# UofgCoastline/EUSIPCO-2026-Robust-Unet

Hardware: NVIDIA B200
Metric: train_images_per_sec (higher is better)
Workload: dtype bf16

## Files before the change

### eusipco-2026-robust-unet_b200/csrc/wgrad_gemm.cu

```cuda
#include "rbu_common.cuh"
#include "rbu_ptx.cuh"
#include "tma_host.cuh"
#include <stdlib.h>

namespace {

constexpr int TILE_PX = 128;
constexpr int BOX_BYTES = TILE_PX * 128;
constexpr int NUM_THREADS = 192;
constexpr int A_STAGES = 2;
constexpr int SMEM_LIMIT = 232448;

struct WParams {
  int N, H, W;
  int TW, TH, TN;
  int tiles_w, tiles_h, tiles_n, tiles_total;
  int Mtot, Ntot, taps, dil, gather;
  int tap_first, tap_end;
  int BM, BN, T;
  int m_blocks, n_blocks, t_groups, ksplit, items;
  int b_stages, tmem_cols;
  float* partial;
};

__device__ __forceinline__ void decode_item(const WParams& p, int item, int& mb, int& nb, int& tg, int& ks) {
  mb = item % p.m_blocks; item /= p.m_blocks;
  nb = item % p.n_blocks; item /= p.n_blocks;
  tg = item % p.t_groups;
  ks = item / p.t_groups;
}
__device__ __forceinline__ void tile_origin(const WParams& p, int tile, int& w0, int& h0, int& n0) {
  w0 = (tile % p.tiles_w) * p.TW;
  tile /= p.tiles_w;
  h0 = (tile % p.tiles_h) * p.TH;
  n0 = (tile / p.tiles_h) * p.TN;
}

__global__ void __launch_bounds__(NUM_THREADS, 1)
wgrad_gemm_kernel(const __grid_constant__ CUtensorMap tmA, const __grid_constant__ CUtensorMap tmB,
                  const __grid_constant__ WParams p) {
  extern __shared__ uint8_t smem_raw[];
  uint8_t* smem = reinterpret_cast<uint8_t*>((reinterpret_cast<uintptr_t>(smem_raw) + 1023) & ~uintptr_t(1023));
  const int a_boxes = p.BM / 64 > 0 ? (p.BM + 63) / 64 : 1;
  const int b_boxes = (p.BN + 63) / 64;
  const int a_bytes = a_boxes * BOX_BYTES;
  const int b_bytes = b_boxes * BOX_BYTES;
  uint8_t* smA = smem;
  uint8_t* smB = smem + A_STAGES * a_bytes;
  uint64_t* bars = reinterpret_cast<uint64_t*>(smB + p.b_stages * b_bytes);
  uint64_t* fullA = bars;
  uint64_t* emptyA = bars + 2;
  uint64_t* fullB = bars + 4;
  uint64_t* emptyB = bars + 12;
  uint64_t* tfull = bars + 20;
  uint64_t* tempty = bars + 21;
  uint32_t* tmem_slot = reinterpret_cast<uint32_t*>(bars + 22);

  const int warp = threadIdx.x >> 5, lane = threadIdx.x & 31;
  if (warp == 0 && lane == 0) {
    ptx::prefetch_tmap(&tmA);
    ptx::prefetch_tmap(&tmB);
  }
  if (warp == 1 && lane == 0) {
    for (int s = 0; s < A_STAGES; ++s) { ptx::mbar_init(&fullA[s], 1); ptx::mbar_init(&emptyA[s], 1); }
    for (int s = 0; s < p.b_stages; ++s) { ptx::mbar_init(&fullB[s], 1); ptx::mbar_init(&emptyB[s], 1); }
    ptx::mbar_init(tfull, 1);
    ptx::mbar_init(tempty, 4);
    ptx::fence_barrier_init();
  }
  if (warp == 2) {
    ptx::tmem_alloc(tmem_slot, (uint32_t)p.tmem_cols);
    ptx::tmem_relinquish();
  }
  ptx::tc_fence_before();
  __syncthreads();
  ptx::tc_fence_after();
  const uint32_t tmem_base = *tmem_slot;

  if (warp == 0) {
    if (lane == 0) {
      int sa = 0, sb = 0;
      uint32_t pha = 0, phb = 0;
      for (int item = blockIdx.x; item < p.items; item += gridDim.x) {
        int mb, nb, tg, ks;
        decode_item(p, item, mb, nb, tg, ks);
        const int t_begin = p.tap_first + tg * p.T;
        const int t_end = min(t_begin + p.T, p.tap_end);
        const int tile0 = (int)((long)ks * p.tiles_total / p.ksplit);
        const int tile1 = (int)((long)(ks + 1) * p.tiles_total / p.ksplit);
        for (int tile = tile0; tile < tile1; ++tile) {
          int w0, h0, n0;
          tile_origin(p, tile, w0, h0, n0);
          {
            const int s = sa;
            const uint32_t ph = pha;
            if (++sa == A_STAGES) { sa = 0; pha ^= 1; }
            ptx::mbar_wait(&emptyA[s], ph ^ 1);
            ptx::mbar_arrive_expect_tx(&fullA[s], (uint32_t)a_bytes);
            for (int bx = 0; bx < a_boxes; ++bx)
              ptx::tma_load_4d(smA + s * a_bytes + bx * BOX_BYTES, &tmA, &fullA[s], mb * p.BM + bx * 64, w0, h0, n0);
          }
          for (int t = t_begin; t < t_end; ++t) {
            const int s = sb;
            const uint32_t ph = phb;
            if (++sb == p.b_stages) { sb = 0; phb ^= 1; }
            ptx::mbar_wait(&emptyB[s], ph ^ 1);
            ptx::mbar_arrive_expect_tx(&fullB[s], (uint32_t)b_bytes);
            for (int bx = 0; bx < b_boxes; ++bx) {
              uint8_t* dst = smB + s * b_bytes + bx * BOX_BYTES;
              const int c0 = nb * p.BN + bx * 64;
              if (p.gather) {
                ptx::tma_load_5d(dst, &tmB, &fullB[s], c0, t & 1, w0, t >> 1, h0);
              } else {
                int dh = 0, dw = 0;
                if (p.taps == 9) { dh = (t / 3 - 1) * p.dil; dw = (t % 3 - 1) * p.dil; }
                ptx::tma_load_4d(dst, &tmB, &fullB[s], c0, w0 + dw, h0 + dh, n0);
              }
            }
          }
        }
      }
    }
  } else if (warp == 1) {
    const uint32_t idesc = ptx::make_idesc_bf16(p.BM, p.BN, 1, 1);
    const uint32_t fullA_s = ptx::smem_u32(fullA), emptyA_s = ptx::smem_u32(emptyA);
    const uint32_t fullB_s = ptx::smem_u32(fullB), emptyB_s = ptx::smem_u32(emptyB);
    const uint32_t hi = ptx::desc_hi(1024);
    const uint32_t a_lo0 = ptx::desc_lo(ptx::smem_u32(smA), BOX_BYTES), b_lo0 = ptx::desc_lo(ptx::smem_u32(smB), BOX_BYTES);
    const uint32_t a_step = (uint32_t)a_bytes >> 4, b_step = (uint32_t)b_bytes >> 4;
    int sa = 0, sb = 0, it = 0;
    uint32_t pha = 0, phb = 0;
    for (int item = blockIdx.x; item < p.items; item += gridDim.x, ++it) {
      int mb, nb, tg, ks;
      decode_item(p, item, mb, nb, tg, ks);
      const int ntap = min(p.tap_first + tg * p.T + p.T, p.tap_end) - (p.tap_first + tg * p.T);
      const int tile0 = (int)((long)ks * p.tiles_total / p.ksplit);
      const int tile1 = (int)((long)(ks + 1) * p.tiles_total / p.ksplit);
      ptx::mbar_wait(tempty, (it & 1) ^ 1);
      ptx::tc_fence_after();
      uint32_t accumulate = 0;
      for (int tile = tile0; tile < tile1; ++tile) {
        ptx::mbar_wait_s(fullA_s + sa * 8, pha);
        ptx::tc_fence_after();
        const uint32_t a_lo = a_lo0 + sa * a_step;
        for (int t = 0; t < ntap; ++t) {
          ptx::mbar_wait_s(fullB_s + sb * 8, phb);
          ptx::tc_fence_after();
          if (ptx::elect_one()) {
            const uint32_t b_lo = b_lo0 + sb * b_step;
            const uint32_t d_tmem = tmem_base + (uint32_t)(t * p.BN);
#pragma unroll
            for (int k = 0; k < TILE_PX / 16; ++k)
              ptx::umma_bf16(d_tmem, ptx::pack_desc(a_lo + k * (2048 >> 4), hi), ptx::pack_desc(b_lo + k * (2048 >> 4), hi),
                             idesc, (k > 0) ? 1u : accumulate);
            ptx::umma_commit_s(emptyB_s + sb * 8);
          }
          __syncwarp();
          if (++sb == p.b_stages) { sb = 0; phb ^= 1; }
        }
        accumulate = 1;
        if (ptx::elect_one()) ptx::umma_commit_s(emptyA_s + sa * 8);
        __syncwarp();
        if (++sa == A_STAGES) { sa = 0; pha ^= 1; }
      }
      if (ptx::elect_one()) ptx::umma_commit(tfull);
      __syncwarp();
    }
  } else {
    const int lg = warp & 3;
    int it = 0;
    for (int item = blockIdx.x; item < p.items; item += gridDim.x, ++it) {
      int mb, nb, tg, ks;
      decode_item(p, item, mb, nb, tg, ks);
      const int t_begin = p.tap_first + tg * p.T;
      const int t_end = min(t_begin + p.T, p.tap_end);
      int m_local;
      bool row_ok;
      if (p.BM == 128) { m_local = lg * 32 + lane; row_ok = true; }
      else { m_local = lg * 16 + lane; row_ok = lane < 16; }
      const int m = mb * p.BM + m_local;
      row_ok = row_ok && (m < p.Mtot);
      ptx::mbar_wait(tfull, it & 1);
      ptx::tc_fence_after();
      const uint32_t t_addr = tmem_base + ((uint32_t)(lg * 32) << 16);
      for (int t = t_begin; t < t_end; ++t) {
        for (int c0 = 0; c0 < p.BN; c0 += 32) {
          uint32_t r[32];
          ptx::tmem_ld_32x32(t_addr + (uint32_t)((t - t_begin) * p.BN + c0), r);
          ptx::tmem_ld_wait();
          const int n0 = nb * p.BN + c0;
          if (row_ok && n0 < p.Ntot) {
            float* dst = p.partial + (((long)ks * p.Mtot + m) * p.taps + t) * p.Ntot + n0;
            if (n0 + 32 <= p.Ntot && (p.Ntot & 3) == 0) {
#pragma unroll
              for (int g = 0; g < 8; ++g)
                *reinterpret_cast<float4*>(dst + g * 4) = make_float4(__uint_as_float(r[g * 4]), __uint_as_float(r[g * 4 + 1]),
                                                                      __uint_as_float(r[g * 4 + 2]), __uint_as_float(r[g * 4 + 3]));
            } else {
              for (int e = 0; e < 32; ++e)
                if (n0 + e < p.Ntot) dst[e] = __uint_as_float(r[e]);
            }
          }
        }
      }
      ptx::tc_fence_before();
      __syncwarp();
      if (lane == 0) ptx::mbar_arrive(tempty);
    }
  }
  ptx::tc_fence_before();
  __syncthreads();
  if (warp == 2) ptx::tmem_dealloc(tmem_base, (uint32_t)p.tmem_cols);
}

template <int NCH>
__global__ void __launch_bounds__(256)
wgrad_reduce_kernel(const float* __restrict__ partial, int ksplit, int Mtot, int taps, int Ntot,
                    float* __restrict__ out, int accumulate, int tap_first, int tap_end) {
  constexpr int KL = 256 / NCH;
  constexpr int MAXT = 9;
  __shared__ float lane_sum[KL][MAXT][NCH + 1];
  __shared__ float res[NCH * MAXT];
  const int nchunks = (Ntot + NCH - 1) / NCH;
  const int m = blockIdx.x / nchunks, n0 = (blockIdx.x - m * nchunks) * NCH;
  const int nn = threadIdx.x % NCH, kl = threadIdx.x / NCH;
  const int n = n0 + nn;
  const long total = (long)Mtot * taps * Ntot;
  float acc[MAXT][2];
#pragma unroll
  for (int t = 0; t < MAXT; ++t) acc[t][0] = acc[t][1] = 0.f;
  if (n < Ntot) {
    const float* src = partial + (long)m * taps * Ntot + n;
    int k = kl;
    for (; k + KL < ksplit; k += 2 * KL) {
#pragma unroll
      for (int t = 0; t < MAXT; ++t)
        if (t >= tap_first && t < tap_end) {
          acc[t][0] += __ldg(src + (long)k * total + (long)t * Ntot);
          acc[t][1] += __ldg(src + (long)(k + KL) * total + (long)t * Ntot);
        }
    }
    if (k < ksplit) {
#pragma unroll
      for (int t = 0; t < MAXT; ++t)
        if (t >= tap_first && t < tap_end) acc[t][0] += __ldg(src + (long)k * total + (long)t * Ntot);
    }
  }
#pragma unroll
  for (int t = 0; t < MAXT; ++t)
    if (t < taps) lane_sum[kl][t][nn] = acc[t][0] + acc[t][1];
  __syncthreads();
  for (int i = threadIdx.x; i < NCH * taps; i += 256) {
    const int t = i / NCH, c = i - t * NCH;
    float sum = lane_sum[0][t][c];
    for (int j = 1; j < KL; ++j) sum += lane_sum[j][t][c];
    res[c * taps + t] = sum;
  }
  __syncthreads();
  const int nw = min(NCH, Ntot - n0);
  float* o = out + ((long)m * Ntot + n0) * taps;
  for (int i = threadIdx.x; i < nw * taps; i += 256) {
    const int t = i % taps;
    if (t >= tap_first && t < tap_end) o[i] = accumulate ? o[i] + res[i] : res[i];
  }
}

bool use_halo(const rbu_wgrad_args* a) {
  static int no_halo = -1;
  if (no_halo < 0) no_halo = getenv("RBU_NO_HALO") ? 1 : 0;
  return !no_halo && rbu_wgrad_halo_supported(a);
}

int pow2ceil_w(int v) {
  int r = 1;
  while (r < v) r <<= 1;
  return r;
}

struct Plan {
  WParams p;
  size_t ws_bytes;
};

int make_plan(const rbu_wgrad_args* a, Plan* pl, int tap_first = 0, int tap_end = -1) {
  WParams& p = pl->p;
  memset(&p, 0, sizeof(p));
  p.tap_first = tap_first;
  p.tap_end = tap_end < 0 ? a->taps : tap_end;
  p.N = a->N; p.H = a->H; p.W = a->W;
  p.gather = a->gather;
  p.taps = a->taps;
  p.dil = a->taps == 9 ? a->dil : 0;
  p.Mtot = a->Ca;
  p.Ntot = a->Cb;
  p.TW = pow2ceil_w(a->W) < 16 ? pow2ceil_w(a->W) : 16;
  if (a->gather) {
    p.TH = TILE_PX / p.TW;
    p.TN = 1;
    p.tiles_w = rbu_cdiv(a->W, p.TW);
    p.tiles_h = rbu_cdiv((long)a->N * a->H, p.TH);
    p.tiles_n = 1;
  } else {
    const int th_max = TILE_PX / p.TW;
    p.TH = pow2ceil_w(a->H) < th_max ? pow2ceil_w(a->H) : th_max;
    p.TN = TILE_PX / (p.TW * p.TH);
    p.tiles_w = rbu_cdiv(a->W, p.TW);
    p.tiles_h = rbu_cdiv(a->H, p.TH);
    p.tiles_n = rbu_cdiv(a->N, p.TN);
  }
  p.tiles_total = p.tiles_w * p.tiles_h * p.tiles_n;
  p.BM = a->Ca > 64 ? 128 : 64;
  p.BN = a->Cb > 64 ? 128 : 64;
  p.T = a->taps == 9 ? 3 : a->taps;
  p.m_blocks = rbu_cdiv(a->Ca, p.BM);
  p.n_blocks = rbu_cdiv(a->Cb, p.BN);
  p.t_groups = rbu_cdiv(p.tap_end - p.tap_first, p.T);
  const int base_items = p.m_blocks * p.n_blocks * p.t_groups;
  int ks = rbu_cdiv(2L * rbu_num_sms(), base_items);
  if (ks > p.tiles_total) ks = p.tiles_total;
  if (ks < 1) ks = 1;
  p.ksplit = ks;
  p.items = base_items * ks;
  const int a_bytes = ((p.BM + 63) / 64) * BOX_BYTES, b_bytes = ((p.BN + 63) / 64) * BOX_BYTES;
  p.b_stages = (SMEM_LIMIT - 2048 - A_STAGES * a_bytes) / b_bytes;
  if (p.b_stages > 8) p.b_stages = 8;
  p.tmem_cols = 32;
  while (p.tmem_cols < p.T * p.BN) p.tmem_cols <<= 1;
  pl->ws_bytes = (size_t)ks * a->Ca * a->taps * a->Cb * sizeof(float);
  return 0;
}

int check_args(const rbu_wgrad_args* a) {
  RBU_CHECK_ARG(a != nullptr, "rbu_wgrad_gemm: null args");
  RBU_CHECK_ARG(a->N > 0 && a->H > 0 && a->W > 0, "rbu_wgrad_gemm: bad pixel grid");
  RBU_CHECK_ARG(a->Ca > 0 && a->Ca % 8 == 0 && a->Cb > 0 && a->Cb % 8 == 0, "rbu_wgrad_gemm: channel counts must be multiples of 8");
  RBU_CHECK_ARG(a->a_ld % 8 == 0 && a->b_ld % 8 == 0, "rbu_wgrad_gemm: ld must be a multiple of 8");
  if (a->gather) RBU_CHECK_ARG(a->taps == 4, "rbu_wgrad_gemm: gather needs taps == 4");
  else RBU_CHECK_ARG(a->taps == 1 || (a->taps == 9 && a->dil >= 1), "rbu_wgrad_gemm: taps must be 1 or 9 (dil >= 1)");
  return RBU_OK;
}

}

void rbu_wgrad_reduce_launch(const float* partial, int ksplit, int Mtot, int taps, int Ntot, float* out, int accumulate,
                             cudaStream_t stream, int tap_first, int tap_end) {
  if (tap_end < 0) tap_end = taps;
  if (Ntot >= 64 && ksplit <= 16)
    wgrad_reduce_kernel<64><<<Mtot * ((Ntot + 63) / 64), 256, 0, stream>>>(partial, ksplit, Mtot, taps, Ntot, out, accumulate, tap_first, tap_end);
  else if (Ntot >= 32 && ksplit <= 64)
    wgrad_reduce_kernel<32><<<Mtot * ((Ntot + 31) / 32), 256, 0, stream>>>(partial, ksplit, Mtot, taps, Ntot, out, accumulate, tap_first, tap_end);
  else
    wgrad_reduce_kernel<16><<<Mtot * ((Ntot + 15) / 16), 256, 0, stream>>>(partial, ksplit, Mtot, taps, Ntot, out, accumulate, tap_first, tap_end);
}

extern "C" size_t rbu_wgrad_workspace_bytes(const rbu_wgrad_args* a) {
  if (check_args(a) != RBU_OK) return 0;
  if (use_halo(a)) return rbu_wgrad_halo_workspace_bytes(a);
  Plan pl;
  make_plan(a, &pl);
  return pl.ws_bytes;
}

size_t rbu_wgrad_generic_workspace_bytes(const rbu_wgrad_args* a, int tap_first, int tap_end) {
  Plan pl;
  make_plan(a, &pl, tap_first, tap_end);
  return pl.ws_bytes;
}

int rbu_wgrad_generic_launch(const rbu_wgrad_args* a, int tap_first, int tap_end, void* workspace, size_t workspace_bytes,
                             cudaStream_t stream) {
  int rc;
  Plan pl;
  make_plan(a, &pl, tap_first, tap_end);
  WParams& p = pl.p;
  RBU_CHECK_ARG(workspace && workspace_bytes >= pl.ws_bytes && ((uintptr_t)workspace & 15) == 0,
                "rbu_wgrad_gemm: workspace too small (%zu < %zu)", workspace_bytes, pl.ws_bytes);
  p.partial = reinterpret_cast<float*>(workspace);

  CUtensorMap tmA, tmB;
  {
    uint64_t dims[4], str[3];
    uint32_t box[4];
    dims[0] = (uint64_t)a->Ca;
    str[0] = (uint64_t)a->a_ld * 2;
    dims[1] = (uint64_t)a->W;
    box[0] = 64; box[1] = (uint32_t)p.TW; box[2] = (uint32_t)p.TH; box[3] = (uint32_t)p.TN;
    if (a->gather) {
      dims[2] = (uint64_t)a->N * a->H; dims[3] = 1;
      str[1] = (uint64_t)a->a_ld * 2 * a->W;
      str[2] = str[1] * dims[2];
    } else {
      dims[2] = (uint64_t)a->H; dims[3] = (uint64_t)a->N;
      str[1] = (uint64_t)a->a_ld * 2 * a->W;
      str[2] = str[1] * a->H;
    }
    rc = rbu_encode_tmap_bf16(&tmA, a->a, 4, dims, str, box);
    if (rc) return rc;
  }
  if (a->gather) {
    const uint64_t dims[5] = {(uint64_t)a->Cb, 2, (uint64_t)a->W, 2, (uint64_t)a->N * a->H};
    const uint64_t str[4] = {(uint64_t)a->b_ld * 2, (uint64_t)a->b_ld * 4, (uint64_t)a->b_ld * 2 * (2 * a->W),
                             (uint64_t)a->b_ld * 4 * (2 * a->W)};
    const uint32_t box[5] = {64, 1, (uint32_t)p.TW, 1, (uint32_t)p.TH};
    rc = rbu_encode_tmap_bf16(&tmB, a->b, 5, dims, str, box);
  } else {
    const uint64_t dims[4] = {(uint64_t)a->Cb, (uint64_t)a->W, (uint64_t)a->H, (uint64_t)a->N};
    const uint64_t str[3] = {(uint64_t)a->b_ld * 2, (uint64_t)a->b_ld * 2 * a->W, (uint64_t)a->b_ld * 2 * a->W * a->H};
    const uint32_t box[4] = {64, (uint32_t)p.TW, (uint32_t)p.TH, (uint32_t)p.TN};
    rc = rbu_encode_tmap_bf16(&tmB, a->b, 4, dims, str, box);
  }
  if (rc) return rc;

  const int a_bytes = ((p.BM + 63) / 64) * BOX_BYTES, b_bytes = ((p.BN + 63) / 64) * BOX_BYTES;
  const int smem_bytes = A_STAGES * a_bytes + p.b_stages * b_bytes + 1024 + 256;
  static std::atomic<unsigned long long> attr_set{0};
  if (rbu_first_use_on_device(&attr_set))
    RBU_CHECK_CUDA(cudaFuncSetAttribute(wgrad_gemm_kernel, cudaFuncAttributeMaxDynamicSharedMemorySize, SMEM_LIMIT));
  const int grid = p.items < rbu_num_sms() ? p.items : rbu_num_sms();
  wgrad_gemm_kernel<<<grid, NUM_THREADS, smem_bytes, stream>>>(tmA, tmB, p);
  RBU_CHECK_LAUNCH();
  rbu_wgrad_reduce_launch(p.partial, p.ksplit, p.Mtot, p.taps, p.Ntot, a->out, a->accumulate, stream, p.tap_first, p.tap_end);
  RBU_CHECK_LAUNCH();
  return RBU_OK;
}

extern "C" int rbu_wgrad_gemm(const rbu_wgrad_args* a, void* workspace, size_t workspace_bytes, void* stream_) {
  cudaStream_t stream = reinterpret_cast<cudaStream_t>(stream_);
  int rc = check_args(a);
  if (rc) return rc;
  RBU_CHECK_ARG(a->a && a->b && a->out && ((uintptr_t)a->a & 15) == 0 && ((uintptr_t)a->b & 15) == 0,
                "rbu_wgrad_gemm: null or misaligned pointer");
  if (use_halo(a)) {
    RBU_CHECK_ARG(workspace && workspace_bytes >= rbu_wgrad_halo_workspace_bytes(a) && ((uintptr_t)workspace & 15) == 0,
                  "rbu_wgrad_gemm: workspace too small");
    return rbu_wgrad_halo_launch(a, workspace, stream);
  }
  return rbu_wgrad_generic_launch(a, 0, -1, workspace, workspace_bytes, stream);
}
```

Before: 1809.

## Double-buffer wgrad TMEM accumulators, widen BN, add direct store, vectorize reduce

The weight-gradient GEMM now keeps two TMEM accumulator slots when they fit, so the epilogue can drain one item while the MMA warp fills the next. It also allows BN=256 with a retuned tap grouping. When split-K is 1 it writes straight to the output and skips both the partial workspace and the reduce kernel. The reduce kernel switches to float4 loads, 64 threads and dynamic shared memory. Risks: the BN=256 tile together with the ksplit heuristic (still computed from the old item count) may leave SMs idle, and the direct path writes to the output with strided scalar stores when taps>1.

```diff
diff --git a/eusipco-2026-robust-unet_b200/csrc/wgrad_gemm.cu b/eusipco-2026-robust-unet_b200/csrc/wgrad_gemm.cu
--- a/eusipco-2026-robust-unet_b200/csrc/wgrad_gemm.cu
+++ b/eusipco-2026-robust-unet_b200/csrc/wgrad_gemm.cu
@@ -20,7 +20,10 @@
   int BM, BN, T;
   int m_blocks, n_blocks, t_groups, ksplit, items;
   int b_stages, tmem_cols;
+  int slots;
+  int direct, accumulate;
   float* partial;
+  float* out;
 };
 
 __device__ __forceinline__ void decode_item(const WParams& p, int item, int& mb, int& nb, int& tg, int& ks) {
@@ -53,8 +56,8 @@
   uint64_t* fullB = bars + 4;
   uint64_t* emptyB = bars + 12;
   uint64_t* tfull = bars + 20;
-  uint64_t* tempty = bars + 21;
-  uint32_t* tmem_slot = reinterpret_cast<uint32_t*>(bars + 22);
+  uint64_t* tempty = bars + 22;
+  uint32_t* tmem_slot = reinterpret_cast<uint32_t*>(bars + 24);
 
   const int warp = threadIdx.x >> 5, lane = threadIdx.x & 31;
   if (warp == 0 && lane == 0) {
@@ -64,8 +67,7 @@
   if (warp == 1 && lane == 0) {
     for (int s = 0; s < A_STAGES; ++s) { ptx::mbar_init(&fullA[s], 1); ptx::mbar_init(&emptyA[s], 1); }
     for (int s = 0; s < p.b_stages; ++s) { ptx::mbar_init(&fullB[s], 1); ptx::mbar_init(&emptyB[s], 1); }
-    ptx::mbar_init(tfull, 1);
-    ptx::mbar_init(tempty, 4);
+    for (int s = 0; s < 2; ++s) { ptx::mbar_init(&tfull[s], 1); ptx::mbar_init(&tempty[s], 4); }
     ptx::fence_barrier_init();
   }
   if (warp == 2) {
@@ -136,8 +138,11 @@
       const int ntap = min(p.tap_first + tg * p.T + p.T, p.tap_end) - (p.tap_first + tg * p.T);
       const int tile0 = (int)((long)ks * p.tiles_total / p.ksplit);
       const int tile1 = (int)((long)(ks + 1) * p.tiles_total / p.ksplit);
-      ptx::mbar_wait(tempty, (it & 1) ^ 1);
+      const int slot = p.slots == 2 ? (it & 1) : 0;
+      const uint32_t use = p.slots == 2 ? (uint32_t)(it >> 1) : (uint32_t)it;
+      ptx::mbar_wait(&tempty[slot], (use & 1) ^ 1);
       ptx::tc_fence_after();
+      const uint32_t acc_base = tmem_base + (uint32_t)(slot * p.T * p.BN);
       uint32_t accumulate = 0;
       for (int tile = tile0; tile < tile1; ++tile) {
         ptx::mbar_wait_s(fullA_s + sa * 8, pha);
@@ -148,7 +153,7 @@
           ptx::tc_fence_after();
           if (ptx::elect_one()) {
             const uint32_t b_lo = b_lo0 + sb * b_step;
-            const uint32_t d_tmem = tmem_base + (uint32_t)(t * p.BN);
+            const uint32_t d_tmem = acc_base + (uint32_t)(t * p.BN);
 #pragma unroll
             for (int k = 0; k < TILE_PX / 16; ++k)
               ptx::umma_bf16(d_tmem, ptx::pack_desc(a_lo + k * (2048 >> 4), hi), ptx::pack_desc(b_lo + k * (2048 >> 4), hi),
@@ -163,7 +168,7 @@
         __syncwarp();
         if (++sa == A_STAGES) { sa = 0; pha ^= 1; }
       }
-      if (ptx::elect_one()) ptx::umma_commit(tfull);
+      if (ptx::elect_one()) ptx::umma_commit(&tfull[slot]);
       __syncwarp();
     }
   } else {
@@ -180,32 +185,58 @@
       else { m_local = lg * 16 + lane; row_ok = lane < 16; }
       const int m = mb * p.BM + m_local;
       row_ok = row_ok && (m < p.Mtot);
-      ptx::mbar_wait(tfull, it & 1);
+      const int slot = p.slots == 2 ? (it & 1) : 0;
+      const uint32_t use = p.slots == 2 ? (uint32_t)(it >> 1) : (uint32_t)it;
+      ptx::mbar_wait(&tfull[slot], use & 1);
       ptx::tc_fence_after();
-      const uint32_t t_addr = tmem_base + ((uint32_t)(lg * 32) << 16);
+      const uint32_t t_addr = tmem_base + ((uint32_t)(lg * 32) << 16) + (uint32_t)(slot * p.T * p.BN);
       for (int t = t_begin; t < t_end; ++t) {
         for (int c0 = 0; c0 < p.BN; c0 += 32) {
           uint32_t r[32];
           ptx::tmem_ld_32x32(t_addr + (uint32_t)((t - t_begin) * p.BN + c0), r);
           ptx::tmem_ld_wait();
           const int n0 = nb * p.BN + c0;
-          if (row_ok && n0 < p.Ntot) {
-            float* dst = p.partial + (((long)ks * p.Mtot + m) * p.taps + t) * p.Ntot + n0;
-            if (n0 + 32 <= p.Ntot && (p.Ntot & 3) == 0) {
-#pragma unroll
-              for (int g = 0; g < 8; ++g)
-                *reinterpret_cast<float4*>(dst + g * 4) = make_float4(__uint_as_float(r[g * 4]), __uint_as_float(r[g * 4 + 1]),
-                                                                      __uint_as_float(r[g * 4 + 2]), __uint_as_float(r[g * 4 + 3]));
+          if (!row_ok || n0 >= p.Ntot) continue;
+          if (p.direct) {
+            float* dst = p.out + ((long)m * p.Ntot + n0) * p.taps + t;
+            if (p.taps == 1 && n0 + 32 <= p.Ntot && (p.Ntot & 3) == 0) {
+              float4* d4 = reinterpret_cast<float4*>(dst);
+#pragma unroll
+              for (int g = 0; g < 8; ++g) {
+                float4 v = make_float4(__uint_as_float(r[g * 4]), __uint_as_float(r[g * 4 + 1]), __uint_as_float(r[g * 4 + 2]),
+                                       __uint_as_float(r[g * 4 + 3]));
+                if (p.accumulate) {
+                  const float4 o = d4[g];
+                  v.x += o.x; v.y += o.y; v.z += o.z; v.w += o.w;
+                }
+                d4[g] = v;
+              }
             } else {
-              for (int e = 0; e < 32; ++e)
-                if (n0 + e < p.Ntot) dst[e] = __uint_as_float(r[e]);
+#pragma unroll
+              for (int e = 0; e < 32; ++e) {
+                if (n0 + e < p.Ntot) {
+                  const float v = __uint_as_float(r[e]);
+                  dst[(long)e * p.taps] = p.accumulate ? dst[(long)e * p.taps] + v : v;
+                }
+              }
             }
+            continue;
+          }
+          float* dst = p.partial + (((long)ks * p.Mtot + m) * p.taps + t) * p.Ntot + n0;
+          if (n0 + 32 <= p.Ntot && (p.Ntot & 3) == 0) {
+#pragma unroll
+            for (int g = 0; g < 8; ++g)
+              *reinterpret_cast<float4*>(dst + g * 4) = make_float4(__uint_as_float(r[g * 4]), __uint_as_float(r[g * 4 + 1]),
+                                                                    __uint_as_float(r[g * 4 + 2]), __uint_as_float(r[g * 4 + 3]));
+          } else {
+            for (int e = 0; e < 32; ++e)
+              if (n0 + e < p.Ntot) dst[e] = __uint_as_float(r[e]);
           }
         }
       }
       ptx::tc_fence_before();
       __syncwarp();
-      if (lane == 0) ptx::mbar_arrive(tempty);
+      if (lane == 0) ptx::mbar_arrive(&tempty[slot]);
     }
   }
   ptx::tc_fence_before();
@@ -214,21 +245,23 @@
 }
 
 template <int NCH>
-__global__ void __launch_bounds__(256)
+__global__ void __launch_bounds__(64)
 wgrad_reduce_kernel(const float* __restrict__ partial, int ksplit, int Mtot, int taps, int Ntot,
                     float* __restrict__ out, int accumulate, int tap_first, int tap_end) {
+  constexpr int NV = NCH / 4;
   constexpr int KL = 256 / NCH;
   constexpr int MAXT = 9;
-  __shared__ float lane_sum[KL][MAXT][NCH + 1];
-  __shared__ float res[NCH * MAXT];
+  extern __shared__ float red_smem[];
+  float* lane_sum = red_smem;
+  float* res = red_smem + KL * taps * (NCH + 1);
   const int nchunks = (Ntot + NCH - 1) / NCH;
   const int m = blockIdx.x / nchunks, n0 = (blockIdx.x - m * nchunks) * NCH;
-  const int nn = threadIdx.x % NCH, kl = threadIdx.x / NCH;
-  const int n = n0 + nn;
+  const int nv = threadIdx.x % NV, kl = threadIdx.x / NV;
+  const int n = n0 + 4 * nv;
   const long total = (long)Mtot * taps * Ntot;
-  float acc[MAXT][2];
-#pragma unroll
-  for (int t = 0; t < MAXT; ++t) acc[t][0] = acc[t][1] = 0.f;
+  float4 acc[MAXT][2];
+#pragma unroll
+  for (int t = 0; t < MAXT; ++t) acc[t][0] = acc[t][1] = make_float4(0.f, 0.f, 0.f, 0.f);
   if (n < Ntot) {
     const float* src = partial + (long)m * taps * Ntot + n;
     int k = kl;
@@ -236,30 +269,41 @@
 #pragma unroll
       for (int t = 0; t < MAXT; ++t)
         if (t >= tap_first && t < tap_end) {
-          acc[t][0] += __ldg(src + (long)k * total + (long)t * Ntot);
-          acc[t][1] += __ldg(src + (long)(k + KL) * total + (long)t * Ntot);
+          const float4 u = __ldg(reinterpret_cast<const float4*>(src + (long)k * total + (long)t * Ntot));
+          const float4 v = __ldg(reinterpret_cast<const float4*>(src + (long)(k + KL) * total + (long)t * Ntot));
+          acc[t][0].x += u.x; acc[t][0].y += u.y; acc[t][0].z += u.z; acc[t][0].w += u.w;
+          acc[t][1].x += v.x; acc[t][1].y += v.y; acc[t][1].z += v.z; acc[t][1].w += v.w;
         }
     }
     if (k < ksplit) {
 #pragma unroll
       for (int t = 0; t < MAXT; ++t)
-        if (t >= tap_first && t < tap_end) acc[t][0] += __ldg(src + (long)k * total + (long)t * Ntot);
+        if (t >= tap_first && t < tap_end) {
+          const float4 u = __ldg(reinterpret_cast<const float4*>(src + (long)k * total + (long)t * Ntot));
+          acc[t][0].x += u.x; acc[t][0].y += u.y; acc[t][0].z += u.z; acc[t][0].w += u.w;
+        }
     }
   }
 #pragma unroll
   for (int t = 0; t < MAXT; ++t)
-    if (t < taps) lane_sum[kl][t][nn] = acc[t][0] + acc[t][1];
+    if (t < taps) {
+      float* ls = lane_sum + (kl * taps + t) * (NCH + 1) + 4 * nv;
+      ls[0] = acc[t][0].x + acc[t][1].x;
+      ls[1] = acc[t][0].y + acc[t][1].y;
+      ls[2] = acc[t][0].z + acc[t][1].z;
+      ls[3] = acc[t][0].w + acc[t][1].w;
+    }
   __syncthreads();
-  for (int i = threadIdx.x; i < NCH * taps; i += 256) {
+  for (int i = threadIdx.x; i < NCH * taps; i += 64) {
     const int t = i / NCH, c = i - t * NCH;
-    float sum = lane_sum[0][t][c];
-    for (int j = 1; j < KL; ++j) sum += lane_sum[j][t][c];
+    float sum = lane_sum[t * (NCH + 1) + c];
+    for (int j = 1; j < KL; ++j) sum += lane_sum[(j * taps + t) * (NCH + 1) + c];
     res[c * taps + t] = sum;
   }
   __syncthreads();
   const int nw = min(NCH, Ntot - n0);
   float* o = out + ((long)m * Ntot + n0) * taps;
-  for (int i = threadIdx.x; i < nw * taps; i += 256) {
+  for (int i = threadIdx.x; i < nw * taps; i += 64) {
     const int t = i % taps;
     if (t >= tap_first && t < tap_end) o[i] = accumulate ? o[i] + res[i] : res[i];
   }
@@ -309,24 +353,29 @@
     p.tiles_n = rbu_cdiv(a->N, p.TN);
   }
   p.tiles_total = p.tiles_w * p.tiles_h * p.tiles_n;
+  const int ntaps = p.tap_end - p.tap_first;
   p.BM = a->Ca > 64 ? 128 : 64;
-  p.BN = a->Cb > 64 ? 128 : 64;
-  p.T = a->taps == 9 ? 3 : a->taps;
+  p.BN = a->Cb > 128 ? 256 : (a->Cb > 64 ? 128 : 64);
+  const int groups = rbu_cdiv(ntaps, 512 / p.BN);
+  p.T = rbu_cdiv(ntaps, groups);
+  p.slots = 2 * p.T * p.BN <= 512 ? 2 : 1;
   p.m_blocks = rbu_cdiv(a->Ca, p.BM);
   p.n_blocks = rbu_cdiv(a->Cb, p.BN);
-  p.t_groups = rbu_cdiv(p.tap_end - p.tap_first, p.T);
+  p.t_groups = rbu_cdiv(ntaps, p.T);
   const int base_items = p.m_blocks * p.n_blocks * p.t_groups;
-  int ks = rbu_cdiv(2L * rbu_num_sms(), base_items);
+  const int a_bytes = ((p.BM + 63) / 64) * BOX_BYTES, b_bytes = ((p.BN + 63) / 64) * BOX_BYTES;
+  const int old_items = rbu_cdiv(a->Ca, p.BM) * rbu_cdiv(a->Cb, a->Cb > 64 ? 128 : 64) * rbu_cdiv(ntaps, a->taps == 9 ? 3 : a->taps);
+  int ks = rbu_cdiv(2L * rbu_num_sms(), old_items);
   if (ks > p.tiles_total) ks = p.tiles_total;
   if (ks < 1) ks = 1;
   p.ksplit = ks;
   p.items = base_items * ks;
-  const int a_bytes = ((p.BM + 63) / 64) * BOX_BYTES, b_bytes = ((p.BN + 63) / 64) * BOX_BYTES;
+  p.direct = ks == 1;
   p.b_stages = (SMEM_LIMIT - 2048 - A_STAGES * a_bytes) / b_bytes;
   if (p.b_stages > 8) p.b_stages = 8;
   p.tmem_cols = 32;
-  while (p.tmem_cols < p.T * p.BN) p.tmem_cols <<= 1;
-  pl->ws_bytes = (size_t)ks * a->Ca * a->taps * a->Cb * sizeof(float);
+  while (p.tmem_cols < p.slots * p.T * p.BN) p.tmem_cols <<= 1;
+  pl->ws_bytes = p.direct ? 0 : (size_t)ks * a->Ca * a->taps * a->Cb * sizeof(float);
   return 0;
 }
 
@@ -345,12 +394,13 @@
 void rbu_wgrad_reduce_launch(const float* partial, int ksplit, int Mtot, int taps, int Ntot, float* out, int accumulate,
                              cudaStream_t stream, int tap_first, int tap_end) {
   if (tap_end < 0) tap_end = taps;
+  auto smem = [taps](int nch) { return (size_t)((256 / nch) * taps * (nch + 1) + nch * taps) * sizeof(float); };
   if (Ntot >= 64 && ksplit <= 16)
-    wgrad_reduce_kernel<64><<<Mtot * ((Ntot + 63) / 64), 256, 0, stream>>>(partial, ksplit, Mtot, taps, Ntot, out, accumulate, tap_first, tap_end);
+    wgrad_reduce_kernel<64><<<Mtot * ((Ntot + 63) / 64), 64, smem(64), stream>>>(partial, ksplit, Mtot, taps, Ntot, out, accumulate, tap_first, tap_end);
   else if (Ntot >= 32 && ksplit <= 64)
-    wgrad_reduce_kernel<32><<<Mtot * ((Ntot + 31) / 32), 256, 0, stream>>>(partial, ksplit, Mtot, taps, Ntot, out, accumulate, tap_first, tap_end);
+    wgrad_reduce_kernel<32><<<Mtot * ((Ntot + 31) / 32), 64, smem(32), stream>>>(partial, ksplit, Mtot, taps, Ntot, out, accumulate, tap_first, tap_end);
   else
-    wgrad_reduce_kernel<16><<<Mtot * ((Ntot + 15) / 16), 256, 0, stream>>>(partial, ksplit, Mtot, taps, Ntot, out, accumulate, tap_first, tap_end);
+    wgrad_reduce_kernel<16><<<Mtot * ((Ntot + 15) / 16), 64, smem(16), stream>>>(partial, ksplit, Mtot, taps, Ntot, out, accumulate, tap_first, tap_end);
 }
 
 extern "C" size_t rbu_wgrad_workspace_bytes(const rbu_wgrad_args* a) {
@@ -373,9 +423,11 @@
   Plan pl;
   make_plan(a, &pl, tap_first, tap_end);
   WParams& p = pl.p;
-  RBU_CHECK_ARG(workspace && workspace_bytes >= pl.ws_bytes && ((uintptr_t)workspace & 15) == 0,
+  RBU_CHECK_ARG(pl.ws_bytes == 0 || (workspace && workspace_bytes >= pl.ws_bytes && ((uintptr_t)workspace & 15) == 0),
                 "rbu_wgrad_gemm: workspace too small (%zu < %zu)", workspace_bytes, pl.ws_bytes);
   p.partial = reinterpret_cast<float*>(workspace);
+  p.out = a->out;
+  p.accumulate = a->accumulate;
 
   CUtensorMap tmA, tmB;
   {
@@ -419,6 +471,7 @@
   const int grid = p.items < rbu_num_sms() ? p.items : rbu_num_sms();
   wgrad_gemm_kernel<<<grid, NUM_THREADS, smem_bytes, stream>>>(tmA, tmB, p);
   RBU_CHECK_LAUNCH();
+  if (p.direct) return RBU_OK;
   rbu_wgrad_reduce_launch(p.partial, p.ksplit, p.Mtot, p.taps, p.Ntot, a->out, a->accumulate, stream, p.tap_first, p.tap_end);
   RBU_CHECK_LAUNCH();
   return RBU_OK;
```

Result: no change. 1822 (median of 6 runs) (+0.7%).
